# quantumjot/sequitr

Hardware: AMD Instinct MI355X
Metric: segmented Mpixels/sec on 512x512 tiles; IoU vs reference (higher is better)
Workload: dtype f32; 1 GPU; U-Net 2-class inference, launches of 32 512x512x1 tiles, fp32 (BASELINE.json configs[1]: filters 16-32-64-128-256, eltwise_mul bridge); logits + uint8 argmax mask; one 32-tile batch per GPU per step; tiles_this_rank=32

## Files before the change

### include/sequitr_hip.h

```cpp
#ifndef SEQUITR_HIP_H
#define SEQUITR_HIP_H

#include <stdint.h>

#ifdef __cplusplus
extern "C" {
#endif

#define SQ_OK 0
#define SQ_EINVAL (-1)
#define SQ_ELAUNCH (-2)
#define SQ_EALIGN (-3)

#define SQ_ACT_NONE 0
#define SQ_ACT_RELU 1
#define SQ_ACT_LEAKY 2

#define SQ_BRIDGE_NONE 0
#define SQ_BRIDGE_ADD 1
#define SQ_BRIDGE_MUL 2
#define SQ_BRIDGE_SUB 3

int sq_version(void);
const char *sq_last_error(void);
// ... 126 lines not shown
int sq_wgan_losses_fwd_f32(const float *Dz, const float *Dx, const float *gn2, float *out2, int N, void *stream);
int sq_wgan_losses_bwd_f32(const float *Dz, const float *Dx, const float *gn2, const float *g_dloss, const float *g_gloss,
                           float *dDz, float *dDx, float *dgn2, int N, void *stream);

int sq_mosaic_pack_f32(const float *x, float *m, int N, int H, int W, int C, int R, int Cc, void *stream);
int sq_mosaic_unpack_f32(const float *m, float *y, int N, int H, int W, int C, int R, int Cc, void *stream);

int64_t sq_dense_workspace_f32(int M, int K, int N);
int sq_dense_fwd_f32(const float *x, const float *w, const float *bias, float *y, float *workspace, int M, int K, int N,
                     float wscale, int act, void *stream);
int sq_dense_wgrad_f32(const float *x, const float *dy, float *dw, float *db, int M, int K, int N, float scale, int accumulate,
                       void *stream);

int64_t sq_wgrad1x1_small_workspace_f32(int64_t npix, int Ca, int Cb);
int sq_wgrad1x1_small_f32(const float *a, const float *b, float *m, float *workspace, int64_t npix, int Ca, int Cb,
                          void *stream);


int sq_conv2d_concat_nhwc_fwd_f32(const float *xa, const float *xb, const float *w, const float *bias, float *y, int N,
                                  int H, int W, int Ca, int Cout, int K, int act, void *stream);

int sq_conv3x3_pool_fwd_f32(const float *x, const float *w, const float *bias, float *y, float *pooled,
                            int N, int H, int W, int Cin, int Cout, int act, void *stream);

int64_t sq_conv_packed_filter_elems_f32(int K, int Cin, int Cout);
int sq_conv_pack_filter_f32(const float *w, float *wp, int K, int Cin, int Cout, void *stream);
int sq_conv_packed_takes_f32(int N, int H, int W, int Cin, int Cout, int K);
int sq_conv2d_packed_nhwc_fwd_f32(const float *x, const float *w, const float *wp, const float *bias, float *y, int N, int H,
                                  int W, int Cin, int Cout, int K, float wscale, int act, void *stream);
int sq_conv3x3_pool_packed_fwd_f32(const float *x, const float *w, const float *wp, const float *bias, float *y, float *pooled,
                                   int N, int H, int W, int Cin, int Cout, int act, void *stream);

int sq_conv_r32_takes_f32(int N, int H, int W, int Cin, int Cout, int K, int act, int pooled);

int sq_conv3x3_head_fwd_f32(const float *x, const float *w, const float *bias, const float *head_w,
                            const float *head_b, float *logits, uint8_t *mask, int N, int H, int W,
                            int Cin, int head_c, int act, void *stream);

int sq_conv3x3_first_block_fwd_f32(const float *x, const float *w1, const float *b1, const float *w2,
                                   const float *b2, float *y, float *pooled, int N, int H, int W,
                                   void *stream);

int sq_convT_conv3x3_fwd_f32(const float *x_low, const float *wt, const float *bt, const float *skip, int bridge,
                             const float *w, const float *bias, float *y, int N, int H, int W, int act, void *stream);


int64_t sq_conv_packed_weights_elems_bf16(int K, int Cin, int Cout);
int sq_conv_pack_weights_bf16(const float *w, void *wp, int K, int Cin, int Cout, float wscale, int transform,
                              void *stream);
int sq_conv_pack_weights_multi_bf16(const float *base, void *out, const int32_t *table, int n_entries,
                                    int total_items, void *stream);
int sq_conv_pack_weights_multi_scaled_bf16(const float *base, void *out, const int32_t *table, const float *scales,
                                           int n_entries, int total_items, void *stream);

int sq_conv2d_nhwc_fwd_bf16(const void *x, const void *wp, const float *bias, void *y, int N, int H, int W,
                            int Cin, int Cout, int K, int act, void *stream);

int sq_conv2d_nhwc_fwd_mixed_f32(const float *x, const void *wp, const float *bias, float *y, int N, int H, int W,
                                 int Cin, int Cout, int K, int act, void *stream);
int sq_conv2d_nhwc_dgrad_actgate_mixed_f32(const float *dy, const void *wp_t, const float *gate, int act, float *dx, int N,
                                           int H, int W, int Cin, int Cout, int K, void *stream);
int sq_conv2d_nhwc_mixed_mosaic_f32(const float *x, const void *wp, const float *bias, const float *gate, float *y, int Nimg,
                                    int h, int w, int Cin, int Cout, int act, int R, int Cc, void *stream);
int64_t sq_conv2d_nhwc_wgrad_workspace_mixed_f32(int N, int H, int W, int Cin, int Cout, int K);
int sq_conv2d_nhwc_wgrad_mixed_f32(const float *x, const float *dy, float *dw, float *db, float *workspace, int N,
                                   int H, int W, int Cin, int Cout, int K, void *stream);
// ... 417 lines not shown
```

### sequitr_amd/_lib.py

```python
import ctypes
import os

_HERE = os.path.dirname(os.path.abspath(__file__))
LIB_PATH = os.path.join(_HERE, "_build", "libsequitr_hip.so")

c_void_p, c_int, c_float, c_int64 = ctypes.c_void_p, ctypes.c_int, ctypes.c_float, ctypes.c_int64


class WgradItem(ctypes.Structure):
    _fields_ = [("x", c_void_p), ("dy", c_void_p), ("dw", c_void_p), ("db", c_void_p),
                ("N", ctypes.c_int32), ("H", ctypes.c_int32), ("W", ctypes.c_int32), ("Cin", ctypes.c_int32),
                ("Cout", ctypes.c_int32), ("K", ctypes.c_int32), ("convT_cout", ctypes.c_int32), ("dw_scale", c_float),
                ("accumulate", ctypes.c_int32), ("mosaic_R", ctypes.c_int32), ("mosaic_Cc", ctypes.c_int32),
                ("reserved", ctypes.c_int32)]

SIGNATURES = {
    "sq_version": (c_int, []),
    "sq_last_error": (ctypes.c_char_p, []),
    "sq_conv2d_nhwc_fwd_f32": (c_int, [c_void_p] * 4 + [c_int] * 6 + [c_float, c_int, c_void_p]),
    "sq_maxpool2x2_fwd_f32": (c_int, [c_void_p] * 2 + [c_int] * 4 + [c_void_p]),
    "sq_avgpool2x2_fwd_f32": (c_int, [c_void_p] * 2 + [c_int] * 4 + [c_void_p]),
    "sq_convT2x2s2_nhwc_fwd_f32": (c_int, [c_void_p] * 5 + [c_int] * 6 + [c_void_p]),
    "sq_bridge_fwd_f32": (c_int, [c_void_p] * 3 + [c_int64, c_int, c_void_p]),
    "sq_conv1x1_argmax_fwd_f32": (c_int, [c_void_p] * 5 + [c_int] * 5 + [c_void_p]),
# ... 123 lines not shown
    "sq_adam_apply_dev_f32": (c_int, [c_void_p] * 4 + [c_int64, c_float, c_float, c_float, c_void_p, c_float, c_void_p]),
    "sq_adam_multi_chunk": (c_int, []),
    "sq_adam_apply_multi_dev_f32": (c_int, [c_void_p, c_int, c_int64, c_float, c_float, c_float, c_void_p, c_float, c_void_p]),
    "sq_pixelnorm_bwd_f32": (c_int, [c_void_p] * 3 + [c_int64, c_int, c_float, c_void_p]),
    "sq_pixelnorm_bwd2_f32": (c_int, [c_void_p] * 5 + [c_int64, c_int, c_float, c_void_p]),
    "sq_pixelnorm_bwd_act_f32": (c_int, [c_void_p] * 3 + [c_int64, c_int, c_float, c_int, c_void_p]),
    "sq_broadcast2x2_act_bwd_f32": (c_int, [c_void_p] * 3 + [c_int] * 4 + [c_float, c_int, c_void_p]),
    "sq_resize_nearest_f32": (c_int, [c_void_p] * 2 + [c_int] * 6 + [c_void_p]),
    "sq_lerp_f32": (c_int, [c_void_p] * 3 + [c_int64, c_int64, c_float, c_void_p, c_void_p]),
    "sq_scale_f32": (c_int, [c_void_p] * 2 + [c_int64, c_int64, c_float, c_void_p, c_int, c_void_p]),
    "sq_act_fwd_f32": (c_int, [c_void_p] * 2 + [c_int64, c_int, c_void_p]),
    "sq_dot_per_sample_workspace_f32": (c_int64, [c_int]),
    "sq_dot_per_sample_f32": (c_int, [c_void_p] * 4 + [c_int, c_int64, c_void_p]),
    "sq_mbstd_fwd_f32": (c_int, [c_void_p] * 3 + [c_int, c_int64, c_void_p]),
    "sq_mbstd_map_workspace": (c_int64, [c_int]),
    "sq_mbstd_map_fwd_f32": (c_int, [c_void_p] * 3 + [c_int, c_int, c_int64, c_int, c_void_p]),
    "sq_mbstd_map_bwd_f32": (c_int, [c_void_p] * 4 + [c_int, c_int, c_int64, c_int, c_void_p]),
    "sq_mbstd_map_bwd2_f32": (c_int, [c_void_p] * 6 + [c_int, c_int, c_int64, c_int, c_void_p]),
    "sq_mbstd_map_fwd_bf16": (c_int, [c_void_p] * 3 + [c_int, c_int, c_int64, c_int, c_void_p]),
    "sq_mbstd_map_bwd_bf16": (c_int, [c_void_p] * 4 + [c_int, c_int, c_int64, c_int, c_void_p]),
    "sq_mbstd_map_bwd2_bf16": (c_int, [c_void_p] * 6 + [c_int, c_int, c_int64, c_int, c_void_p]),
    "sq_wgan_losses_fwd_f32": (c_int, [c_void_p] * 4 + [c_int, c_void_p]),
    "sq_wgan_losses_bwd_f32": (c_int, [c_void_p] * 8 + [c_int, c_void_p]),
    "sq_dense_wgrad_f32": (c_int, [c_void_p] * 4 + [c_int] * 3 + [c_float, c_int, c_void_p]),
    "sq_wgrad1x1_small_workspace_f32": (c_int64, [c_int64, c_int, c_int]),
    "sq_wgrad1x1_small_f32": (c_int, [c_void_p] * 4 + [c_int64, c_int, c_int, c_void_p]),
    "sq_conv2d_concat_nhwc_fwd_f32": (c_int, [c_void_p] * 5 + [c_int] * 7 + [c_void_p]),
    "sq_conv3x3_pool_fwd_f32": (c_int, [c_void_p] * 5 + [c_int] * 6 + [c_void_p]),
    "sq_conv3x3_head_fwd_f32": (c_int, [c_void_p] * 7 + [c_int] * 6 + [c_void_p]),
    "sq_conv_packed_filter_elems_f32": (c_int64, [c_int] * 3),
    "sq_conv_pack_filter_f32": (c_int, [c_void_p] * 2 + [c_int] * 3 + [c_void_p]),
    "sq_conv_packed_takes_f32": (c_int, [c_int] * 6),
    "sq_conv_r32_takes_f32": (c_int, [c_int] * 8),
    "sq_conv2d_packed_nhwc_fwd_f32": (c_int, [c_void_p] * 5 + [c_int] * 6 + [c_float, c_int, c_void_p]),
    "sq_conv3x3_pool_packed_fwd_f32": (c_int, [c_void_p] * 6 + [c_int] * 6 + [c_void_p]),
    "sq_conv3x3_first_block_fwd_f32": (c_int, [c_void_p] * 7 + [c_int] * 3 + [c_void_p]),
    "sq_conv_packed_weights_elems_bf16": (c_int64, [c_int] * 3),
    "sq_conv_pack_weights_bf16": (c_int, [c_void_p] * 2 + [c_int] * 3 + [c_float, c_int, c_void_p]),
    "sq_conv2d_nhwc_fwd_bf16": (c_int, [c_void_p] * 4 + [c_int] * 7 + [c_void_p]),
    "sq_conv2d_nhwc_fwd_mixed_f32": (c_int, [c_void_p] * 4 + [c_int] * 7 + [c_void_p]),
    "sq_conv2d_nhwc_wgrad_workspace_mixed_f32": (c_int64, [c_int] * 6),
    "sq_conv2d_nhwc_wgrad_mixed_f32": (c_int, [c_void_p] * 5 + [c_int] * 6 + [c_void_p]),
    "sq_conv2d_nhwc_wgrad_scaled_mixed_f32": (c_int, [c_void_p] * 5 + [c_int] * 6 + [c_float, c_void_p]),
    "sq_conv2d_nhwc_wgrad_scaled_f32": (c_int, [c_void_p] * 5 + [c_int] * 6 + [c_float, c_void_p]),
    "sq_conv3x3_first_fwd_bf16": (c_int, [c_void_p] * 4 + [c_int] * 6 + [c_void_p]),
    "sq_conv2d_nhwc_wgrad_workspace_bf16": (c_int64, [c_int] * 6),
    "sq_conv2d_nhwc_wgrad_bf16": (c_int, [c_void_p] * 5 + [c_int] * 6 + [c_void_p]),
    "sq_convT2x2s2_wgrad_bf16": (c_int, [c_void_p] * 5 + [c_int] * 5 + [c_void_p]),
    "sq_cast_f32_to_bf16": (c_int, [c_void_p] * 2 + [c_int64, c_void_p]),
    "sq_cast_bf16_to_f32": (c_int, [c_void_p] * 2 + [c_int64, c_void_p]),
    "sq_head_concat_fwd_bf16": (c_int, [c_void_p] * 3 + [c_int64, c_int, c_void_p]),
    "sq_head_concat_bwd_bf16": (c_int, [c_void_p] * 3 + [c_int64, c_int, c_void_p]),
    "sq_maxpool2x2_fwd_bf16": (c_int, [c_void_p] * 2 + [c_int] * 4 + [c_void_p]),
    "sq_maxpool2x2_bwd_bf16": (c_int, [c_void_p] * 3 + [c_int] * 4 + [c_void_p]),
    "sq_conv_pack_weights_multi_bf16": (c_int, [c_void_p, c_void_p, c_void_p, c_int, c_int, c_void_p]),
    "sq_conv_pack_weights_multi_scaled_bf16": (c_int, [c_void_p] * 4 + [c_int, c_int, c_void_p]),
    "sq_conv2d_nhwc_fwd_dropout_bf16": (c_int, [c_void_p] * 4 + [c_int] * 7 + [c_float, ctypes.c_uint32, c_void_p, c_void_p]),
    "sq_conv3x3_first_fwd_mask_bf16": (c_int, [c_void_p] * 5 + [c_int] * 6 + [c_void_p]),
    "sq_conv2d_nhwc_fwd_mask_bf16": (c_int, [c_void_p] * 5 + [c_int] * 7 + [c_void_p]),
    "sq_conv2d_nhwc_dgrad_maskgate_bf16": (c_int, [c_void_p] * 3 + [c_float, c_void_p] + [c_int] * 6 + [c_void_p]),
    "sq_conv2d_nhwc_wgrad_mixed_mosaic_f32": (c_int, [c_void_p] * 5 + [c_int] * 7 + [c_float, c_void_p]),
    "sq_conv2d_nhwc_mixed_mosaic_f32": (c_int, [c_void_p] * 5 + [c_int] * 8 + [c_void_p]),
    "sq_conv2d_nhwc_dgrad_actgate_mixed_f32": (c_int, [c_void_p] * 3 + [c_int, c_void_p] + [c_int] * 6 + [c_void_p]),
    "sq_conv2d_nhwc_fwd_dropout_pool_bf16": (c_int, [c_void_p] * 5 + [c_int] * 7 + [c_float, ctypes.c_uint32, c_void_p, c_void_p]),
    "sq_conv3x3_first_block_dropout_pool_bf16": (c_int, [c_void_p] * 9 + [c_int] * 3 + [c_float, ctypes.c_uint32, c_void_p, c_void_p]),
    "sq_relu_scale_bwd_bf16": (c_int, [c_void_p] * 3 + [c_int64, c_float, c_void_p]),
# ... 91 lines not shown
```

### sequitr_amd/csrc/sq_common.h

```cpp
#pragma once
#include <hip/hip_runtime.h>
#include <stdint.h>
#include <stdio.h>
#include "../../include/sequitr_hip.h"

typedef float f32x4 __attribute__((ext_vector_type(4)));

#define SQ_NOT_MINE 1

void sq_set_error(const char *fmt, ...);

#define SQ_REQUIRE(cond, ...)            \
    do {                                 \
        if (!(cond)) {                   \
            sq_set_error(__VA_ARGS__);   \
            return SQ_EINVAL;            \
        }                                \
    } while (0)

int sq_plan_bf16_kc(int Cin);
int sq_plan_bf16_bn(int64_t ntiles, int Cout, bool pn, bool mos);
int sq_plan_mosaic_splitk(int Nimg, int h, int w, int Cin, int Cout, int R, int Cc, bool have_ws, int64_t workspace_bytes);
int sq_plan_f32_bn(int64_t ntiles, int Cout);
bool sq_plan_f32_stage32(int bn, int KS, int KC, int Cin, bool concat);
bool sq_plan_l0_takes(int mode, int cout, int act, int H, int W, bool concat, int head_c, bool pooled);
bool sq_plan_r32_takes(int N, int H, int W, int Cin, int Cout, int K, int act, bool wscale1, bool concat, bool head, bool pooled);
#ifndef SQ_L0_OCC
#define SQ_L0_OCC 4
#endif
#ifndef SQ_L0_UP_OCC
#define SQ_L0_UP_OCC 2
#endif
#ifndef SQ_CT_WNI
#define SQ_CT_WNI 1
#endif
constexpr int SQ_CT_BM = 128;
constexpr int sq_l0_occ(bool up, int nb) { return up ? SQ_L0_UP_OCC : (nb == 2 ? 2 : SQ_L0_OCC); }
constexpr int sq_v2_occ(int bn, int kc, bool up) { return up ? 3 : ((bn >= 64 || kc == 32) ? 2 : (bn >= 32 ? 3 : 4)); }
constexpr int sq_ct_occ(int wni) { return wni == 4 ? 2 : (wni == 2 ? 3 : 4); }
int sq_plan_l0_grid(int ntiles, int occ);
void sq_plan_tile_stride(int G, int tiles_x, int tiles_y, int *gx, int *gy, int *gn);
int sq_plan_v2_grid(int ntiles, int cblocks, int occ, int *tiles_per_block);
int sq_plan_ct_wni();
bool sq_plan_ct_takes(int N, int H, int W, int Cin, int Cout);
int sq_plan_ct_grid(int total, int mtiles, int occ);
int sq_wgrad_f32_plan(int N, int H, int W, int Cin, int Cout, int K, int64_t *out);

#define SQ_ALIGNED16(p) ((((uintptr_t)(p)) & 15u) == 0)

#define SQ_REQUIRE_ALIGNED(p)                                     \
    do {                                                          \
        if (!SQ_ALIGNED16(p)) {                                   \
            sq_set_error("%s: pointer %s not 16-byte aligned", __func__, #p); \
            return SQ_EALIGN;                                     \
        }                                                         \
    } while (0)

template <int C>
// ... 102 lines not shown
```

### sequitr_amd/csrc/sq_conv_f32_l0.hip

```cpp
#include <stdlib.h>
#include "sq_common.h"
#include "sq_conv_epi.h"

#ifndef SQ_L0_SETPRIO
#define SQ_L0_SETPRIO 1
#endif

namespace {

constexpr int TH = 16, TW = 16, HWD = 18, HP = HWD * HWD;
constexpr int PS = 24;
constexpr int XS_FLOATS = HP * PS;
constexpr int XITEMS = HP * 4, XSLOTS = 6;
constexpr int IN_W = 20, IN_FLOATS = IN_W * IN_W;
constexpr int UP_W = 10, UP_CIN = 32, UP_PS = 40, UP_FLOATS = UP_W * UP_W * UP_PS;
constexpr unsigned OOB = 0x80000000u;

enum { EPI_STORE = 0, EPI_POOL = 1, EPI_HEAD = 2 };
enum { M_PLAIN = 0, M_FIRST = 1, M_UP = 2 };

struct L0Args {
    const float *x, *w, *bias;
    float *y;
    int N, H, W;
    int tiles_x, tiles_y, ntiles;
    int gx, gy, gn;
    SqConvEpi epi;
};

struct Pos { int tx, ty, n; };

typedef unsigned u32x4 __attribute__((__vector_size__(4 * sizeof(unsigned))));
typedef unsigned u32x2 __attribute__((__vector_size__(2 * sizeof(unsigned))));

__device__ __forceinline__ void row_transpose(float &a0, float &a1, float &a2, float &a3) {
    const auto p = __builtin_amdgcn_permlane16_swap(__float_as_uint(a0), __float_as_uint(a1), false, false);
    const auto q = __builtin_amdgcn_permlane16_swap(__float_as_uint(a2), __float_as_uint(a3), false, false);
    const auto u = __builtin_amdgcn_permlane32_swap(p[0], q[0], false, false);
    const auto v = __builtin_amdgcn_permlane32_swap(p[1], q[1], false, false);
    a0 = __uint_as_float(u[0]); a2 = __uint_as_float(u[1]);
    a1 = __uint_as_float(v[0]); a3 = __uint_as_float(v[1]);
}

__device__ __forceinline__ float relu(float v) { return __builtin_fmaxf(v, 0.0f); }

template <int MODE, int EPI, int BRIDGE, int NB>
__global__ __launch_bounds__(256, sq_l0_occ(MODE == M_UP, NB)) void conv_l0_kernel(const L0Args a) {
    static_assert(NB == 1 || (NB == 2 && MODE == M_PLAIN && EPI == EPI_STORE), "32 output channels: the plain form only");
    constexpr int CO = 16 * NB;
    extern __shared__ __attribute__((aligned(16))) float smem[];
    float *xs = smem;
    float *xin = smem + XS_FLOATS;
    float *xl = smem + XS_FLOATS;

    const int tid = threadIdx.x, lane = tid & 63, wv = tid >> 6;
    const int li = lane & 15, kk = lane >> 4;
    const int H = a.H, W = a.W;
    const int G = (int)gridDim.x;
    const int vb = (int)sq_xcd_remap(blockIdx.x, gridDim.x);
    if (vb >= a.ntiles) return;
    const int t_count = (a.ntiles - vb + G - 1) / G;

    const __amdgpu_buffer_rsrc_t xrsrc = __builtin_amdgcn_make_buffer_rsrc(
        const_cast<float *>(a.x), 0, (int)((size_t)a.N * H * W * (MODE == M_FIRST ? 1 : 16) * 4), 0x00020000);
    const __amdgpu_buffer_rsrc_t yrsrc = __builtin_amdgcn_make_buffer_rsrc(
        a.y, 0, a.y ? (int)((size_t)a.N * H * W * CO * 4) : 0, 0x00020000);

    float af[9][4][NB];
#pragma unroll
    for (int t = 0; t < 9; ++t)
#pragma unroll
        for (int s = 0; s < 4; ++s)
#pragma unroll
            for (int nb = 0; nb < NB; ++nb) af[t][s][nb] = a.w[(t * 16 + 4 * s + kk) * CO + nb * 16 + li];
    float4 bv[NB];
#pragma unroll
    for (int nb = 0; nb < NB; ++nb)
        bv[nb] = a.bias ? *reinterpret_cast<const float4 *>(a.bias + nb * 16 + 4 * kk) : make_float4(0.f, 0.f, 0.f, 0.f);

    auto decode = [&](int tile) {
        Pos p;
// ... 226 lines not shown
#pragma unroll
                for (int t = 0; t < 2; ++t) {
                    const float4 q = bl[t][s8 >> 2];
                    const float b = (s8 & 3) == 0 ? q.x : ((s8 & 3) == 1 ? q.y : ((s8 & 3) == 2 ? q.z : q.w));
                    c1[t] = __builtin_amdgcn_mfma_f32_16x16x4f32(aw[s8], b, s8 == 0 ? (f32x4){0.f, 0.f, 0.f, 0.f} : c1[t], 0, 0, 0);
                }
            }
#pragma unroll
            for (int t = 0; t < 2; ++t) {
                const int blk = bp + t;
                const float u[4] = {c1[t][0] + upb.x, c1[t][1] + upb.y, c1[t][2] + upb.z, c1[t][3] + upb.w};
                const float sk[4] = {sr[blk].x, sr[blk].y, sr[blk].z, sr[blk].w};
                float m[4];
#pragma unroll
                for (int e = 0; e < 4; ++e)
                    m[e] = BRIDGE == SQ_BRIDGE_ADD ? u[e] + sk[e]
                         : (BRIDGE == SQ_BRIDGE_MUL ? u[e] * sk[e] : (BRIDGE == SQ_BRIDGE_SUB ? u[e] - sk[e] : u[e]));
                if (!inner) {
                    const int j = blk * 16 + li, jc = j < 81 ? j : 80;
                    const int hy = 2 * (jc / 9) + (((wv >> 1) + 1) & 1), hx = 2 * (jc % 9) + (((wv & 1) + 1) & 1);
                    const int gy = p.ty * TH - 1 + hy, gx = p.tx * TW - 1 + hx;
                    const bool inside = (unsigned)gy < (unsigned)H && (unsigned)gx < (unsigned)W;
#pragma unroll
                    for (int e = 0; e < 4; ++e) m[e] = inside ? m[e] : 0.f;
                }
                row_transpose(m[0], m[1], m[2], m[3]);
                if ((upk[blk] >> 16) != 0xFFFFu) *reinterpret_cast<float4 *>(xs + (upk[blk] >> 16)) = make_float4(m[0], m[1], m[2], m[3]);
            }
        }
    };

    f32x4 acc[4][NB];
    const float *xb = xs + ((4 * wv) * HWD + li) * PS + 4 * kk;
    auto mfma_phase = [&]() {
        float4 bq[2][3];
#pragma unroll
        for (int kx = 0; kx < 3; ++kx) bq[0][kx] = *reinterpret_cast<const float4 *>(xb + kx * PS);
#if SQ_L0_SETPRIO
        __builtin_amdgcn_s_setprio(0);
#endif
#pragma unroll
        for (int h = 0; h < 6; ++h) {
            if (h + 1 < 6) {
#pragma unroll
                for (int kx = 0; kx < 3; ++kx)
                    bq[(h + 1) & 1][kx] = *reinterpret_cast<const float4 *>(xb + ((h + 1) * HWD + kx) * PS);
            }
            __builtin_amdgcn_sched_barrier(0);
#pragma unroll
            for (int kx = 0; kx < 3; ++kx) {
                const float4 q = bq[h & 1][kx];
                const float b[4] = {q.x, q.y, q.z, q.w};
#pragma unroll
                for (int s = 0; s < 4; ++s) {
#pragma unroll
                    for (int ky = 2; ky >= 0; --ky) {
                        const int r = h - ky;
                        if (r < 0 || r > 3) continue;
                        const bool first = ky == 0 && kx == 0 && s == 0;
#pragma unroll
                        for (int nb = 0; nb < NB; ++nb)
                            acc[r][nb] = __builtin_amdgcn_mfma_f32_16x16x4f32(af[ky * 3 + kx][s][nb], b[s],
                                                                              first ? (f32x4){0.f, 0.f, 0.f, 0.f} : acc[r][nb], 0, 0, 0);
                    }
                }
            }
            __builtin_amdgcn_sched_barrier(0);
        }
#if SQ_L0_SETPRIO
        __builtin_amdgcn_s_setprio(3);
#endif
    };

    const int yvoff = (((4 * wv) * W + li) * CO + 4 * kk) * 4;
    const __amdgpu_buffer_rsrc_t prsrc = __builtin_amdgcn_make_buffer_rsrc(
        a.epi.pooled, 0, EPI == EPI_POOL ? (int)((size_t)a.N * Hl * Wl * 16 * 4) : 0, 0x00020000);
    const int pvoff = (((2 * wv) * Wl + (li >> 1)) * 16 + 4 * kk) * 4;
    float *hws = smem + XS_FLOATS;
    float hb0 = 0.f, hb1 = 0.f;
    const __amdgpu_buffer_rsrc_t grsrc = __builtin_amdgcn_make_buffer_rsrc(
        a.epi.logits, 0, EPI == EPI_HEAD ? (int)((size_t)a.N * H * W * 2 * 4) : 0, 0x00020000);
    const __amdgpu_buffer_rsrc_t mrsrc = __builtin_amdgcn_make_buffer_rsrc(
        a.epi.mask, 0, (EPI == EPI_HEAD && a.epi.mask) ? (int)((size_t)a.N * H * W) : 0, 0x00020000);
    const int gvoff = ((4 * wv + kk) * W + li) * 8, mvoff = (4 * wv + kk) * W + li;
    if constexpr (EPI == EPI_HEAD) {
        static_assert(MODE == M_PLAIN, "the head table sits right behind the halo image");
        if (tid < 64) hws[tid] = (tid >> 4) < 2 ? a.epi.head_w[(tid & 15) * 2 + (tid >> 4)] : 0.f;
        if (a.epi.head_b) { hb0 = a.epi.head_b[0]; hb1 = a.epi.head_b[1]; }
    }
    auto epilogue = [&](const Pos &p) {
        if constexpr (NB > 1) {
            const int tbase = (((p.n * H + p.ty * TH) * W + p.tx * TW) * CO) * 4;
#pragma unroll
            for (int r = 0; r < 4; ++r)
#pragma unroll
                for (int nb = 0; nb < NB; ++nb) {
                    const f32x4 t = (f32x4){relu(acc[r][nb][0] + bv[nb].x), relu(acc[r][nb][1] + bv[nb].y),
                                            relu(acc[r][nb][2] + bv[nb].z), relu(acc[r][nb][3] + bv[nb].w)};
                    __builtin_amdgcn_raw_buffer_store_b128(*reinterpret_cast<const u32x4 *>(&t), yrsrc,
// ... 23 lines not shown
#pragma unroll
                for (int j = 0; j < 4; ++j) {
                    const float v = __builtin_fmaxf(o[2 * pr][j], o[2 * pr + 1][j]);
                    const float u = __builtin_bit_cast(float, __builtin_amdgcn_mov_dpp(__builtin_bit_cast(int, v), 0xB1, 0xF, 0xF, true));
                    mp[j] = __builtin_fmaxf(u, v);
                }
                __builtin_amdgcn_raw_buffer_store_b128(*reinterpret_cast<const u32x4 *>(&mp), prsrc,
                                                       (li & 1) ? (int)OOB : pvoff + pbase + pr * Wl * 64, 0, 0);
            }
        }
        if constexpr (EPI == EPI_HEAD) {
#pragma unroll
            for (int j = 0; j < 4; ++j) row_transpose(o[0][j], o[1][j], o[2][j], o[3][j]);
            float4 hq[4];
#pragma unroll
            for (int r = 0; r < 4; ++r) hq[r] = *reinterpret_cast<const float4 *>(hws + (lane & 3) * 16 + 4 * r);
            f32x4 z = (f32x4){0.f, 0.f, 0.f, 0.f};
#pragma unroll
            for (int r = 0; r < 4; ++r) {
                const float hv[4] = {hq[r].x, hq[r].y, hq[r].z, hq[r].w};
#pragma unroll
                for (int j = 0; j < 4; ++j) z = __builtin_amdgcn_mfma_f32_4x4x1f32(hv[j], o[r][j], z, 0, 0, 0);
            }
            const float z0 = z[0], z1 = z[1];
            const float v0 = a.epi.head_b ? z0 + hb0 : z0, v1 = a.epi.head_b ? z1 + hb1 : z1;
            const int pbase = (p.n * H + p.ty * TH) * W + p.tx * TW;
            const float lg[2] = {v0, v1};
            __builtin_amdgcn_raw_buffer_store_b64(*reinterpret_cast<const u32x2 *>(lg), grsrc, gvoff, pbase * 8, 0);
            __builtin_amdgcn_raw_buffer_store_b8((unsigned char)(v1 > v0 ? 1 : 0), mrsrc, mvoff, pbase, 0);
        }
    };

    Pos cur = decode(vb), nxt = cur, nn = cur;
    if constexpr (MODE == M_PLAIN) {
        issue_halo(cur);
        __builtin_amdgcn_s_waitcnt(0x0F70);
        commit_halo();
        __syncthreads();
        for (int it = 0; it < t_count; ++it) {
            const bool has_next = it + 1 < t_count;
            if (has_next) { nxt = advance(cur); issue_halo(nxt); }
            mfma_phase();
            __builtin_amdgcn_s_waitcnt(0x0F70);
            if (has_next) {
                __syncthreads();
                commit_halo();
            }
            epilogue(cur);
            if (has_next) __syncthreads();
            cur = nxt;
        }
    }
    if constexpr (MODE == M_FIRST) {
        issue_patch(cur);
        __builtin_amdgcn_s_waitcnt(0x0F70);
        commit_patch(0);
        __syncthreads();
        first_conv(cur, 0);
        if (t_count > 1) {
            nxt = advance(cur);
            issue_patch(nxt);
            __builtin_amdgcn_s_waitcnt(0x0F70);
            commit_patch(1);
        }
        __syncthreads();
        for (int it = 0; it < t_count; ++it) {
            const bool has_next = it + 1 < t_count, has_next2 = it + 2 < t_count;
            if (has_next2) { nn = advance(nxt); issue_patch(nn); }
            mfma_phase();
            __builtin_amdgcn_s_waitcnt(0x0F70);
            if (has_next) {
                __syncthreads();
                first_conv(nxt, (it + 1) & 1);
            }
            if (has_next2) commit_patch(it & 1);
            epilogue(cur);
            if (has_next) __syncthreads();
            cur = nxt;
            nxt = nn;
        }
    }
    if constexpr (MODE == M_UP) {
        issue_low(cur);
        issue_skip(cur);
        __builtin_amdgcn_s_waitcnt(0x0F70);
        commit_low();
        if (t_count > 1) { nxt = advance(cur); issue_low(nxt); }
        __syncthreads();
        up_conv(cur);
        __builtin_amdgcn_s_waitcnt(0x0F70);
        __syncthreads();
        for (int it = 0; it < t_count; ++it) {
            const bool has_next = it + 1 < t_count, has_next2 = it + 2 < t_count;
            if (has_next) { commit_low(); issue_skip(nxt); }
            if (has_next2) { nn = advance(nxt); issue_low(nn); }
            mfma_phase();
            __builtin_amdgcn_s_waitcnt(0x0F70);
            if (has_next) {
                __syncthreads();
                up_conv(nxt);
            }
            epilogue(cur);
            if (has_next) __syncthreads();
            cur = nxt;
            nxt = nn;
        }
    }
}

template <int MODE, int EPI, int BRIDGE = 0, int NB = 1>
int launch_l0(const L0Args &a0, hipStream_t st) {
    static bool attr_set = false;
    auto kern = conv_l0_kernel<MODE, EPI, BRIDGE, NB>;
    constexpr int lds = (XS_FLOATS + (MODE == M_FIRST ? 2 * IN_FLOATS : (MODE == M_UP ? UP_FLOATS : 0)) + (EPI == EPI_HEAD ? 64 : 0)) * 4;
    if (!attr_set) {
        if (hipFuncSetAttribute(reinterpret_cast<const void *>(kern), hipFuncAttributeMaxDynamicSharedMemorySize, lds) != hipSuccess) {
            sq_set_error("conv_l0: cannot reserve %d bytes of LDS", lds);
            return SQ_ELAUNCH;
        }
        attr_set = true;
    }
    L0Args a = a0;
    a.tiles_x = a.W / TW;
    a.tiles_y = a.H / TH;
    a.ntiles = a.tiles_x * a.tiles_y * a.N;
    const int G = sq_plan_l0_grid(a.ntiles, sq_l0_occ(MODE == M_UP, NB));
    sq_plan_tile_stride(G, a.tiles_x, a.tiles_y, &a.gx, &a.gy, &a.gn);
    hipLaunchKernelGGL(kern, dim3(G), dim3(256), lds, st, a);
    return sq_check_launch("conv_l0");
}

}

int sq_conv_l0_launch(int mode, const float *x, const float *w, const float *bias, float *y, int N, int H, int W,
                      int cout, int act, const SqConvEpi &epi, hipStream_t st) {
    if (!sq_plan_l0_takes(mode, cout, act, H, W, epi.x2 != nullptr, epi.head_w ? epi.head_c : 0,
                          epi.pooled != nullptr))
        return SQ_L0_NOT_MINE;
    L0Args a = {};
    a.x = x; a.w = w; a.bias = bias; a.y = y; a.N = N; a.H = H; a.W = W; a.epi = epi;
    const int e = epi.head_w ? EPI_HEAD : (epi.pooled ? EPI_POOL : EPI_STORE);
    if (mode == M_PLAIN) {
        if (e == EPI_HEAD) return launch_l0<M_PLAIN, EPI_HEAD>(a, st);
        if (e == EPI_POOL) return launch_l0<M_PLAIN, EPI_POOL>(a, st);
        if (cout == 32) return launch_l0<M_PLAIN, EPI_STORE, 0, 2>(a, st);
        return launch_l0<M_PLAIN, EPI_STORE>(a, st);
    }
    if (mode == M_FIRST) {
        if (e == EPI_HEAD) return SQ_L0_NOT_MINE;
        if (e == EPI_POOL) return launch_l0<M_FIRST, EPI_POOL>(a, st);
        return launch_l0<M_FIRST, EPI_STORE>(a, st);
    }
    if (mode == M_UP) {
        if (e != EPI_STORE) return SQ_L0_NOT_MINE;
        switch (epi.up_bridge) {
            case SQ_BRIDGE_ADD: return launch_l0<M_UP, EPI_STORE, SQ_BRIDGE_ADD>(a, st);
            case SQ_BRIDGE_MUL: return launch_l0<M_UP, EPI_STORE, SQ_BRIDGE_MUL>(a, st);
            case SQ_BRIDGE_SUB: return launch_l0<M_UP, EPI_STORE, SQ_BRIDGE_SUB>(a, st);
            default: return launch_l0<M_UP, EPI_STORE, SQ_BRIDGE_NONE>(a, st);
        }
    }
    return SQ_L0_NOT_MINE;
}
```

### sequitr_amd/csrc/sq_conv_plan.hip

```cpp
#include "sq_conv_epi.h"
#include <stdlib.h>

namespace {
constexpr int TILE = 16;
int64_t ntiles_of(int N, int H, int W) { return (int64_t)((W + TILE - 1) / TILE) * ((H + TILE - 1) / TILE) * N; }
}

int sq_plan_bf16_kc(int Cin) { return Cin % 32 == 0 ? 32 : (Cin % 16 == 0 ? 16 : 8); }

int sq_plan_bf16_bn(int64_t ntiles, int Cout, bool pn, bool mos) {
    if (pn) return Cout <= 16 ? 16 : (Cout <= 32 ? 32 : 64);
    int bn = Cout >= 64 ? 64 : (Cout > 16 ? 32 : 16);
    static const int narrow = [] { const char *e = getenv("SQ_CONV_BF16_NARROW"); return e ? atoi(e) : 1; }();
    while (narrow && bn > 16 && ntiles * ((Cout + bn - 1) / bn) < 2 * 256) bn >>= 1;
    static const int force_bn = [] { const char *e = getenv("SQ_MOS_BN"); return e ? atoi(e) : 0; }();
    if (mos && (force_bn == 16 || force_bn == 32 || force_bn == 64) && force_bn <= ((Cout + 15) / 16) * 16) bn = force_bn;
    return bn;
}

int sq_plan_mosaic_splitk(int Nimg, int h, int w, int Cin, int Cout, int R, int Cc, bool have_ws, int64_t workspace_bytes) {
    const int H = R * (h + 1), W = Cc * (w + 1);
    const int nchunk = Cin / sq_plan_bf16_kc(Cin);
    const int64_t blocks = ntiles_of(1, H, W) * ((Cout + 15) / 16);
    const int64_t slice = (int64_t)Nimg * h * w * Cout * 4;
    int S = 1;
    static const int sk_on = [] { const char *e = getenv("SQ_CONV_SPLITK"); return e ? atoi(e) : 1; }();
    if (sk_on && have_ws && Cout % 4 == 0 && blocks < 256 && nchunk >= 4)
        while (S < 8 && nchunk % (2 * S) == 0 && nchunk / (2 * S) >= 2 && blocks * S < 512 && slice * 2 * S <= workspace_bytes) S *= 2;
    static const int force_s = [] { const char *e = getenv("SQ_MOS_S"); return e ? atoi(e) : 0; }();
    if (force_s >= 1 && have_ws && nchunk % force_s == 0 && slice * force_s <= workspace_bytes) S = force_s;
    return S;
}

int sq_plan_f32_bn(int64_t ntiles, int Cout) {
    int bn = Cout >= 64 ? 64 : (Cout > 16 ? 32 : 16);
    while (bn > 16 && ntiles * ((Cout + bn - 1) / bn) < 2 * 256) bn >>= 1;
    return bn;
}

bool sq_plan_f32_stage32(int bn, int KS, int KC, int Cin, bool concat) {
    static const bool on = [] { const char *e = getenv("SQ_CONV_STAGE32"); return !(e && e[0] == '0'); }();
    return KS == 3 && KC == 16 && bn == 32 && Cin % 32 == 0 && !concat && on;
}

bool sq_plan_l0_takes(int mode, int cout, int act, int H, int W, bool concat, int head_c, bool pooled) {
    if (cout != 16 && !(cout == 32 && mode == 0 && !head_c && !pooled)) return false;
    const char *e = getenv("SQ_CONV_L0");
    if (e && e[0] == '0') return false;
    if (act != SQ_ACT_RELU || H % 16 != 0 || W % 16 != 0 || concat) return false;
    if (head_c && head_c != 2) return false;
    if (head_c && pooled) return false;
    return true;
}

bool sq_plan_r32_takes(int N, int H, int W, int Cin, int Cout, int K, int act, bool wscale1, bool concat, bool head, bool pooled) {
    (void)pooled;
    if (K != 3 || Cin != 32 || Cout != 32 || !wscale1 || act != SQ_ACT_RELU || concat || head) return false;
    if (N <= 0 || H <= 0 || W <= 0 || H % 16 != 0 || W % 16 != 0) return false;
    const char *e = getenv("SQ_CONV_R32");
    if (e && e[0] == '0') return false;
    if ((size_t)N * H * W * 32 * 4 >= ((size_t)1 << 31)) return false;
    const int bn = sq_plan_f32_bn(ntiles_of(N, H, W), Cout);
    return bn == 32 && sq_plan_f32_stage32(bn, K, 16, Cin, concat);
}

extern "C" int sq_conv_r32_takes_f32(int N, int H, int W, int Cin, int Cout, int K, int act, int pooled) {
    return sq_plan_r32_takes(N, H, W, Cin, Cout, K, act, true, false, false, pooled != 0) ? 1 : 0;
}

int sq_plan_l0_grid(int ntiles, int occ) {
    const int want = 256 * occ;
    return ntiles < want ? ntiles : want;
}

void sq_plan_tile_stride(int G, int tiles_x, int tiles_y, int *gx, int *gy, int *gn) {
    const int per_image = tiles_x * tiles_y;
    *gn = G / per_image;
    *gy = (G % per_image) / tiles_x;
    *gx = (G % per_image) % tiles_x;
}

int sq_plan_v2_grid(int ntiles, int cblocks, int occ, int *tiles_per_block) {
    int want = (256 * occ + cblocks - 1) / cblocks;
    if (want < 1) want = 1;
    int tpb = (ntiles + want - 1) / want;
// ... 174 lines not shown
```

### sequitr_amd/ops.py

```python
import os

import torch

from . import _lib

ACT = {None: 0, "none": 0, "relu": 1, "leaky": 2}
BRIDGE = {None: 0, "none": 0, "eltwise_add": 1, "eltwise_mul": 2, "eltwise_sub": 3}


def _stream():
    return torch.cuda.current_stream().cuda_stream


def _chk(t, name, dtype=torch.float32, ndim=None):
    if not isinstance(t, torch.Tensor):
        raise TypeError("%s must be a torch.Tensor" % name)
    if not t.is_cuda:
        raise _lib.SequitrHipError("%s must live in GPU memory (no CPU fallback exists)" % name)
    if t.dtype != dtype:
        raise TypeError("%s must be %s, got %s" % (name, dtype, t.dtype))
    if not t.is_contiguous():
        raise ValueError("%s must be contiguous (NHWC)" % name)
    if ndim is not None and t.dim() != ndim:
        raise ValueError("%s must have %d dims, got %s" % (name, ndim, tuple(t.shape)))
# ... 170 lines not shown
        self.repack()

    def repack(self):
        K, _, Cin, Cout = self.w.shape
        self.epoch = invalidation_epoch()
        _lib.check(_lib.load().sq_conv_pack_filter_f32(_ptr(self.w), _ptr(self.wp), K, Cin, Cout, _stream()),
                   "sq_conv_pack_filter_f32")

    def current(self, w):
        if w is not self.w:
            raise ValueError("pack= belongs to another filter tensor than the call's w")
        if self.epoch != invalidation_epoch():
            self.repack()
        return self.wp


def pack_filter(w):
    if w.dim() != 4 or w.shape[0] != w.shape[1] or w.dtype != torch.float32:
        return None
    if _lib.load().sq_conv_packed_filter_elems_f32(w.shape[0], w.shape[2], w.shape[3]) <= 0:
        return None
    return FilterPackF32(w)


def conv_packed_takes(x_shape, w_shape):
    N, H, W, Cin = x_shape
    return bool(_lib.load().sq_conv_packed_takes_f32(N, H, W, Cin, w_shape[3], w_shape[0])) and w_shape[2] == Cin


def conv_r32_takes(x_shape, w_shape, act="relu", pooled=False):
    N, H, W, Cin = x_shape
    return bool(_lib.load().sq_conv_r32_takes_f32(N, H, W, Cin, w_shape[3], w_shape[0], ACT[act], 1 if pooled else 0)) \
        and w_shape[2] == Cin


def _packed_filter(w, K, Cin, Cout, wscale, transform):
    for plan in list(_PLANS):
        wp = plan.lookup(w, K, Cin, Cout, wscale, transform)
        if wp is not None:
            return wp
    cacheable = w.is_leaf and w.requires_grad
    key = (w.data_ptr(), K, Cin, Cout, float(wscale), bool(transform))
    if cacheable and key in _PACKS:
        return _PACKS[key][1]
    lib = _lib.load()
    n = lib.sq_conv_packed_weights_elems_bf16(K, Cin, Cout)
    wp = torch.empty((n,), dtype=torch.bfloat16, device=w.device)
    _lib.check(lib.sq_conv_pack_weights_bf16(_ptr(w), _ptr(wp), K, Cin, Cout, float(wscale), 1 if transform else 0,
                                            _stream()), "sq_conv_pack_weights_bf16")
    if cacheable:
        _PACKS[key] = (w, wp)
    return wp


def _conv2d_mixed(x, w, bias, act, wscale, y, transform):
    N, H, W, Cin = x.shape
    K, Cout = w.shape[0], (w.shape[2] if transform else w.shape[3])
    lib = _lib.load()
    wp = _packed_filter(w, K, Cin, Cout, wscale, transform)
    _lib.check(lib.sq_conv2d_nhwc_fwd_mixed_f32(_ptr(x), _ptr(wp), _ptr(bias), _ptr(y), N, H, W, Cin, Cout, K, ACT[act],
                                               _stream()), "sq_conv2d_nhwc_fwd_mixed_f32")
    return y


def dense(x, w, bias=None, act=None, wscale=1.0):
    _chk(x, "x", ndim=2), _chk(w, "w", ndim=2)
# ... 1319 lines not shown
```

Measured before the change: 1720 Mpixels/s.

## Defer l0 conv tile epilogue stores into next tile's MFMA phase

Adds a DEFER variant of the level-0 conv kernel. The bias+ReLU+store (and the pool) of the previous tile's output rows is interleaved into the MFMA steps of the next tile through an after_step hook, and halo/patch/skip prefetches move to later MFMA steps. The aim is to hide global store latency and epilogue ALU work behind matrix math. It is on by default for up-mode and 32-channel plain convs, and an env var can force it on or off. This adds register pressure, since one accumulator set is kept live across tiles.

```diff
diff --git a/include/sequitr_hip.h b/include/sequitr_hip.h
--- a/include/sequitr_hip.h
+++ b/include/sequitr_hip.h
@@ -182,6 +182,8 @@
                                    int N, int H, int W, int Cin, int Cout, int act, void *stream);
 
 int sq_conv_r32_takes_f32(int N, int H, int W, int Cin, int Cout, int K, int act, int pooled);
+
+int sq_conv_l0_defers_f32(int mode, int epi_kind, int cout);
 
 int sq_conv3x3_head_fwd_f32(const float *x, const float *w, const float *bias, const float *head_w,
                             const float *head_b, float *logits, uint8_t *mask, int N, int H, int W,
diff --git a/sequitr_amd/_lib.py b/sequitr_amd/_lib.py
--- a/sequitr_amd/_lib.py
+++ b/sequitr_amd/_lib.py
@@ -179,6 +179,7 @@
     "sq_conv_pack_filter_f32": (c_int, [c_void_p] * 2 + [c_int] * 3 + [c_void_p]),
     "sq_conv_packed_takes_f32": (c_int, [c_int] * 6),
     "sq_conv_r32_takes_f32": (c_int, [c_int] * 8),
+    "sq_conv_l0_defers_f32": (c_int, [c_int] * 3),
     "sq_conv2d_packed_nhwc_fwd_f32": (c_int, [c_void_p] * 5 + [c_int] * 6 + [c_float, c_int, c_void_p]),
     "sq_conv3x3_pool_packed_fwd_f32": (c_int, [c_void_p] * 6 + [c_int] * 6 + [c_void_p]),
     "sq_conv3x3_first_block_fwd_f32": (c_int, [c_void_p] * 7 + [c_int] * 3 + [c_void_p]),
diff --git a/sequitr_amd/csrc/sq_common.h b/sequitr_amd/csrc/sq_common.h
--- a/sequitr_amd/csrc/sq_common.h
+++ b/sequitr_amd/csrc/sq_common.h
@@ -24,6 +24,7 @@
 int sq_plan_f32_bn(int64_t ntiles, int Cout);
 bool sq_plan_f32_stage32(int bn, int KS, int KC, int Cin, bool concat);
 bool sq_plan_l0_takes(int mode, int cout, int act, int H, int W, bool concat, int head_c, bool pooled);
+bool sq_plan_l0_defers(int mode, int epi_kind, int cout);
 bool sq_plan_r32_takes(int N, int H, int W, int Cin, int Cout, int K, int act, bool wscale1, bool concat, bool head, bool pooled);
 #ifndef SQ_L0_OCC
 #define SQ_L0_OCC 4
diff --git a/sequitr_amd/csrc/sq_conv_f32_l0.hip b/sequitr_amd/csrc/sq_conv_f32_l0.hip
--- a/sequitr_amd/csrc/sq_conv_f32_l0.hip
+++ b/sequitr_amd/csrc/sq_conv_f32_l0.hip
@@ -44,9 +44,10 @@
 
 __device__ __forceinline__ float relu(float v) { return __builtin_fmaxf(v, 0.0f); }
 
-template <int MODE, int EPI, int BRIDGE, int NB>
+template <int MODE, int EPI, int BRIDGE, int NB, bool DEFER>
 __global__ __launch_bounds__(256, sq_l0_occ(MODE == M_UP, NB)) void conv_l0_kernel(const L0Args a) {
     static_assert(NB == 1 || (NB == 2 && MODE == M_PLAIN && EPI == EPI_STORE), "32 output channels: the plain form only");
+    static_assert(!(DEFER && EPI == EPI_HEAD), "the head's epilogue needs all 16 accumulators of the previous tile");
     constexpr int CO = 16 * NB;
     extern __shared__ __attribute__((aligned(16))) float smem[];
     float *xs = smem;
@@ -339,7 +340,7 @@
 
     f32x4 acc[4][NB];
     const float *xb = xs + ((4 * wv) * HWD + li) * PS + 4 * kk;
-    auto mfma_phase = [&]() {
+    auto mfma_phase = [&](auto &&after_step) {
         float4 bq[2][3];
 #pragma unroll
         for (int kx = 0; kx < 3; ++kx) bq[0][kx] = *reinterpret_cast<const float4 *>(xb + kx * PS);
@@ -372,6 +373,7 @@
                     }
                 }
             }
+            after_step(h);
             __builtin_amdgcn_sched_barrier(0);
         }
 #if SQ_L0_SETPRIO
@@ -461,7 +463,8 @@
     };
 
     Pos cur = decode(vb), nxt = cur, nn = cur;
-    if constexpr (MODE == M_PLAIN) {
+    auto nothing = [](int) {};
+    if constexpr (MODE == M_PLAIN && !DEFER) {
         issue_halo(cur);
         __builtin_amdgcn_s_waitcnt(0x0F70);
         commit_halo();
@@ -469,7 +472,7 @@
         for (int it = 0; it < t_count; ++it) {
             const bool has_next = it + 1 < t_count;
             if (has_next) { nxt = advance(cur); issue_halo(nxt); }
-            mfma_phase();
+            mfma_phase(nothing);
             __builtin_amdgcn_s_waitcnt(0x0F70);
             if (has_next) {
                 __syncthreads();
@@ -480,7 +483,7 @@
             cur = nxt;
         }
     }
-    if constexpr (MODE == M_FIRST) {
+    if constexpr (MODE == M_FIRST && !DEFER) {
         issue_patch(cur);
         __builtin_amdgcn_s_waitcnt(0x0F70);
         commit_patch(0);
@@ -496,7 +499,7 @@
         for (int it = 0; it < t_count; ++it) {
             const bool has_next = it + 1 < t_count, has_next2 = it + 2 < t_count;
             if (has_next2) { nn = advance(nxt); issue_patch(nn); }
-            mfma_phase();
+            mfma_phase(nothing);
             __builtin_amdgcn_s_waitcnt(0x0F70);
             if (has_next) {
                 __syncthreads();
@@ -509,7 +512,7 @@
             nxt = nn;
         }
     }
-    if constexpr (MODE == M_UP) {
+    if constexpr (MODE == M_UP && !DEFER) {
         issue_low(cur);
         issue_skip(cur);
         __builtin_amdgcn_s_waitcnt(0x0F70);
@@ -523,7 +526,7 @@
             const bool has_next = it + 1 < t_count, has_next2 = it + 2 < t_count;
             if (has_next) { commit_low(); issue_skip(nxt); }
             if (has_next2) { nn = advance(nxt); issue_low(nn); }
-            mfma_phase();
+            mfma_phase(nothing);
             __builtin_amdgcn_s_waitcnt(0x0F70);
             if (has_next) {
                 __syncthreads();
@@ -535,12 +538,151 @@
             nxt = nn;
         }
     }
+
+    if constexpr (DEFER) {
+        f32x4 pa0[NB];
+#pragma unroll
+        for (int nb = 0; nb < NB; ++nb) pa0[nb] = (f32x4){0.f, 0.f, 0.f, 0.f};
+        auto store_pair = [&](int pr, int ybase, int pbase) {
+            float o[2][NB][4];
+#pragma unroll
+            for (int rr = 0; rr < 2; ++rr)
+#pragma unroll
+                for (int nb = 0; nb < NB; ++nb) {
+                    const f32x4 v = (pr == 0 && rr == 0) ? pa0[nb] : acc[2 * pr + rr][nb];
+                    o[rr][nb][0] = relu(v[0] + bv[nb].x); o[rr][nb][1] = relu(v[1] + bv[nb].y);
+                    o[rr][nb][2] = relu(v[2] + bv[nb].z); o[rr][nb][3] = relu(v[3] + bv[nb].w);
+                }
+#pragma unroll
+            for (int rr = 0; rr < 2; ++rr)
+#pragma unroll
+                for (int nb = 0; nb < NB; ++nb) {
+                    const f32x4 t = (f32x4){o[rr][nb][0], o[rr][nb][1], o[rr][nb][2], o[rr][nb][3]};
+                    __builtin_amdgcn_raw_buffer_store_b128(*reinterpret_cast<const u32x4 *>(&t), yrsrc,
+                                                           ybase + (2 * pr + rr) * W * CO * 4 + nb * 64, 0, 0);
+                }
+            if constexpr (EPI == EPI_POOL) {
+                f32x4 mp;
+#pragma unroll
+                for (int j = 0; j < 4; ++j) {
+                    const float v = __builtin_fmaxf(o[0][0][j], o[1][0][j]);
+                    const float u = __builtin_bit_cast(float, __builtin_amdgcn_mov_dpp(__builtin_bit_cast(int, v), 0xB1, 0xF, 0xF, true));
+                    mp[j] = __builtin_fmaxf(u, v);
+                }
+                __builtin_amdgcn_raw_buffer_store_b128(*reinterpret_cast<const u32x4 *>(&mp), prsrc, pbase + pr * Wl * 64, 0, 0);
+            }
+        };
+        Pos prev = cur;
+        bool pend = false;
+        auto prev_ybase = [&]() {
+            const int tbase = (((prev.n * H + prev.ty * TH) * W + prev.tx * TW) * CO) * 4;
+            return pend ? yvoff + tbase : (int)OOB;
+        };
+        auto prev_pbase = [&]() {
+            const int pb = (((prev.n * Hl + prev.ty * (TH / 2)) * Wl + prev.tx * (TW / 2)) * 16) * 4;
+            return (pend && !(li & 1)) ? pvoff + pb : (int)OOB;
+        };
+        auto retire = [&]() {
+#pragma unroll
+            for (int nb = 0; nb < NB; ++nb) pa0[nb] = acc[0][nb];
+            prev = cur;
+            pend = true;
+        };
+        if constexpr (MODE == M_PLAIN) {
+            issue_halo(cur);
+            __builtin_amdgcn_s_waitcnt(0x0F70);
+            commit_halo();
+            __syncthreads();
+            for (int it = 0; it < t_count; ++it) {
+                const bool has_next = it + 1 < t_count;
+                nxt = advance(cur);
+                const int ybase = prev_ybase(), pbase = prev_pbase();
+                mfma_phase([&](int h) {
+                    if (h < 2) store_pair(h, ybase, pbase);
+                    if (h == 3 && has_next) issue_halo(nxt);
+                });
+                retire();
+                __builtin_amdgcn_s_waitcnt(0x0F70);
+                if (has_next) {
+                    __syncthreads();
+                    commit_halo();
+                    __syncthreads();
+                }
+                cur = nxt;
+            }
+        }
+        if constexpr (MODE == M_FIRST) {
+            issue_patch(cur);
+            __builtin_amdgcn_s_waitcnt(0x0F70);
+            commit_patch(0);
+            __syncthreads();
+            first_conv(cur, 0);
+            if (t_count > 1) {
+                nxt = advance(cur);
+                issue_patch(nxt);
+                __builtin_amdgcn_s_waitcnt(0x0F70);
+                commit_patch(1);
+            }
+            __syncthreads();
+            for (int it = 0; it < t_count; ++it) {
+                const bool has_next = it + 1 < t_count, has_next2 = it + 2 < t_count;
+                nn = advance(nxt);
+                const int ybase = prev_ybase(), pbase = prev_pbase();
+                mfma_phase([&](int h) {
+                    if (h < 2) store_pair(h, ybase, pbase);
+                    if (h == 3 && has_next2) issue_patch(nn);
+                });
+                retire();
+                __builtin_amdgcn_s_waitcnt(0x0F70);
+                if (has_next) {
+                    __syncthreads();
+                    first_conv(nxt, (it + 1) & 1);
+                }
+                if (has_next2) commit_patch(it & 1);
+                if (has_next) __syncthreads();
+                cur = nxt;
+                nxt = nn;
+            }
+        }
+        if constexpr (MODE == M_UP) {
+            issue_low(cur);
+            issue_skip(cur);
+            __builtin_amdgcn_s_waitcnt(0x0F70);
+            commit_low();
+            if (t_count > 1) { nxt = advance(cur); issue_low(nxt); }
+            __syncthreads();
+            up_conv(cur);
+            __builtin_amdgcn_s_waitcnt(0x0F70);
+            __syncthreads();
+            for (int it = 0; it < t_count; ++it) {
+                const bool has_next = it + 1 < t_count, has_next2 = it + 2 < t_count;
+                nn = advance(nxt);
+                const int ybase = prev_ybase(), pbase = prev_pbase();
+                mfma_phase([&](int h) {
+                    if (h < 2) store_pair(h, ybase, pbase);
+                    if (h == 1 && has_next) commit_low();
+                    if (h == 3 && has_next) issue_skip(nxt);
+                    if (h == 4 && has_next2) issue_low(nn);
+                });
+                retire();
+                __builtin_amdgcn_s_waitcnt(0x0F70);
+                if (has_next) {
+                    __syncthreads();
+                    up_conv(nxt);
+                    __syncthreads();
+                }
+                cur = nxt;
+                nxt = nn;
+            }
+        }
+        epilogue(prev);
+    }
 }
 
-template <int MODE, int EPI, int BRIDGE = 0, int NB = 1>
+template <int MODE, int EPI, int BRIDGE = 0, int NB = 1, bool DEFER = false>
 int launch_l0(const L0Args &a0, hipStream_t st) {
     static bool attr_set = false;
-    auto kern = conv_l0_kernel<MODE, EPI, BRIDGE, NB>;
+    auto kern = conv_l0_kernel<MODE, EPI, BRIDGE, NB, DEFER>;
     constexpr int lds = (XS_FLOATS + (MODE == M_FIRST ? 2 * IN_FLOATS : (MODE == M_UP ? UP_FLOATS : 0)) + (EPI == EPI_HEAD ? 64 : 0)) * 4;
     if (!attr_set) {
         if (hipFuncSetAttribute(reinterpret_cast<const void *>(kern), hipFuncAttributeMaxDynamicSharedMemorySize, lds) != hipSuccess) {
@@ -569,24 +711,25 @@
     L0Args a = {};
     a.x = x; a.w = w; a.bias = bias; a.y = y; a.N = N; a.H = H; a.W = W; a.epi = epi;
     const int e = epi.head_w ? EPI_HEAD : (epi.pooled ? EPI_POOL : EPI_STORE);
+    const bool defer = sq_plan_l0_defers(mode, e, cout);
     if (mode == M_PLAIN) {
         if (e == EPI_HEAD) return launch_l0<M_PLAIN, EPI_HEAD>(a, st);
-        if (e == EPI_POOL) return launch_l0<M_PLAIN, EPI_POOL>(a, st);
-        if (cout == 32) return launch_l0<M_PLAIN, EPI_STORE, 0, 2>(a, st);
-        return launch_l0<M_PLAIN, EPI_STORE>(a, st);
+        if (e == EPI_POOL) return defer ? launch_l0<M_PLAIN, EPI_POOL, 0, 1, true>(a, st) : launch_l0<M_PLAIN, EPI_POOL>(a, st);
+        if (cout == 32) return defer ? launch_l0<M_PLAIN, EPI_STORE, 0, 2, true>(a, st) : launch_l0<M_PLAIN, EPI_STORE, 0, 2>(a, st);
+        return defer ? launch_l0<M_PLAIN, EPI_STORE, 0, 1, true>(a, st) : launch_l0<M_PLAIN, EPI_STORE>(a, st);
     }
     if (mode == M_FIRST) {
         if (e == EPI_HEAD) return SQ_L0_NOT_MINE;
-        if (e == EPI_POOL) return launch_l0<M_FIRST, EPI_POOL>(a, st);
-        return launch_l0<M_FIRST, EPI_STORE>(a, st);
+        if (e == EPI_POOL) return defer ? launch_l0<M_FIRST, EPI_POOL, 0, 1, true>(a, st) : launch_l0<M_FIRST, EPI_POOL>(a, st);
+        return defer ? launch_l0<M_FIRST, EPI_STORE, 0, 1, true>(a, st) : launch_l0<M_FIRST, EPI_STORE>(a, st);
     }
     if (mode == M_UP) {
         if (e != EPI_STORE) return SQ_L0_NOT_MINE;
         switch (epi.up_bridge) {
-            case SQ_BRIDGE_ADD: return launch_l0<M_UP, EPI_STORE, SQ_BRIDGE_ADD>(a, st);
-            case SQ_BRIDGE_MUL: return launch_l0<M_UP, EPI_STORE, SQ_BRIDGE_MUL>(a, st);
-            case SQ_BRIDGE_SUB: return launch_l0<M_UP, EPI_STORE, SQ_BRIDGE_SUB>(a, st);
-            default: return launch_l0<M_UP, EPI_STORE, SQ_BRIDGE_NONE>(a, st);
+            case SQ_BRIDGE_ADD: return defer ? launch_l0<M_UP, EPI_STORE, SQ_BRIDGE_ADD, 1, true>(a, st) : launch_l0<M_UP, EPI_STORE, SQ_BRIDGE_ADD>(a, st);
+            case SQ_BRIDGE_MUL: return defer ? launch_l0<M_UP, EPI_STORE, SQ_BRIDGE_MUL, 1, true>(a, st) : launch_l0<M_UP, EPI_STORE, SQ_BRIDGE_MUL>(a, st);
+            case SQ_BRIDGE_SUB: return defer ? launch_l0<M_UP, EPI_STORE, SQ_BRIDGE_SUB, 1, true>(a, st) : launch_l0<M_UP, EPI_STORE, SQ_BRIDGE_SUB>(a, st);
+            default: return defer ? launch_l0<M_UP, EPI_STORE, SQ_BRIDGE_NONE, 1, true>(a, st) : launch_l0<M_UP, EPI_STORE, SQ_BRIDGE_NONE>(a, st);
         }
     }
     return SQ_L0_NOT_MINE;
diff --git a/sequitr_amd/csrc/sq_conv_plan.hip b/sequitr_amd/csrc/sq_conv_plan.hip
--- a/sequitr_amd/csrc/sq_conv_plan.hip
+++ b/sequitr_amd/csrc/sq_conv_plan.hip
@@ -51,6 +51,21 @@
     if (head_c && head_c != 2) return false;
     if (head_c && pooled) return false;
     return true;
+}
+
+bool sq_plan_l0_defers(int mode, int epi_kind, int cout) {
+    if (mode < 0 || mode > 2 || epi_kind < 0 || epi_kind > 2 || (cout != 16 && cout != 32)) return false;
+    if (epi_kind == 2) return false;
+    if (cout == 32 && !(mode == 0 && epi_kind == 0)) return false;
+    if (mode == 2 && epi_kind != 0) return false;
+    const char *e = getenv("SQ_L0_DEFER");
+    if (e && e[0] == '0') return false;
+    if (e && e[0] == '2') return true;
+    return mode == 2 || cout == 32;
+}
+
+extern "C" int sq_conv_l0_defers_f32(int mode, int epi_kind, int cout) {
+    return sq_plan_l0_defers(mode, epi_kind, cout) ? 1 : 0;
 }
 
 bool sq_plan_r32_takes(int N, int H, int W, int Cin, int Cout, int K, int act, bool wscale1, bool concat, bool head, bool pooled) {
diff --git a/sequitr_amd/ops.py b/sequitr_amd/ops.py
--- a/sequitr_amd/ops.py
+++ b/sequitr_amd/ops.py
@@ -226,6 +226,14 @@
     N, H, W, Cin = x_shape
     return bool(_lib.load().sq_conv_r32_takes_f32(N, H, W, Cin, w_shape[3], w_shape[0], ACT[act], 1 if pooled else 0)) \
         and w_shape[2] == Cin
+
+
+L0_MODE = {"plain": 0, "first": 1, "up": 2}
+L0_EPI = {"store": 0, "pool": 1, "head": 2}
+
+
+def conv_l0_defers(mode, epi_kind, cout=16):
+    return bool(_lib.load().sq_conv_l0_defers_f32(L0_MODE.get(mode, mode), L0_EPI.get(epi_kind, epi_kind), cout))
 
 
 def _packed_filter(w, K, Cin, Cout, wscale, transform):
```

Result: no change. 1732 Mpixels/s, median of 6 (+0.7%).
